# gmlwns2000/sea-attention

Measured on AMD Instinct MI355X. Metric: tokens/sec + achieved HBM GB/s, OPT-1.3B SEA T=4096 k=64, 1/2/4/8 MI355X, higher is better.
Workload: dtype bf16

## Files before the change

sea-attention_amd/csrc/sea_topk.hip:

```cpp
#include "sea_common.hpp"
#include "sea_tail.hpp"
#include "sea_convfrag.hpp"


#ifdef SEA_STAMP
__device__ unsigned long long sea_dbg[16];
#define STAMP(i) do { if (threadIdx.x == 0) { unsigned long long _t = __builtin_amdgcn_s_memtime(); \
  atomicAdd(&sea_dbg[i], _t - _tprev); _tprev = _t; } } while (0)
#else
#define STAMP(i) do {} while (0)
#endif

namespace sea {

constexpr int TK_THREADS = 256;
constexpr int TK_WAVES = TK_THREADS / WAVE;
constexpr int TK_MAX_BINS = 2048;

__device__ inline uint32_t f2key(float f) {
  f = f + 0.0f;
  uint32_t u = __float_as_uint(f);
  return u ^ ((u >> 31) ? 0xFFFFFFFFu : 0x80000000u);
}

struct TopkParams {
  const void* src;
  int64_t sn, sh, st;
  int H, T_dst, T_m, T_src;
  int is_causal, max_k;
  int M;
  int nchunks;
  int W;
  int G;
  const int32_t* keep;
  int64_t keep_stride_n;
  uint32_t* bits;
  float* mask_out;
  int32_t* row_nnz;
  int32_t* head_off;
  const int32_t* t_src_dev;
  int t_src_stride;
  int32_t* crow1;
};

template <typename T> __device__ inline void load4(const T* p, float* f);
template <> __device__ inline void load4<float>(const float* p, float* f) {
  float4 v = *reinterpret_cast<const float4*>(p);
  f[0] = v.x; f[1] = v.y; f[2] = v.z; f[3] = v.w;
}
template <> __device__ inline void load4<__hip_bfloat16>(const __hip_bfloat16* p, float* f) {
  uint2 v = *reinterpret_cast<const uint2*>(p);
  f[0] = __uint_as_float(v.x << 16); f[1] = __uint_as_float(v.x & 0xffff0000u);
  f[2] = __uint_as_float(v.y << 16); f[3] = __uint_as_float(v.y & 0xffff0000u);
}
template <> __device__ inline void load4<__half>(const __half* p, float* f) {
  uint2 v = *reinterpret_cast<const uint2*>(p);
  const __half2* h = reinterpret_cast<const __half2*>(&v);
  float2 a = __half22float2(h[0]), b = __half22float2(h[1]);
  f[0] = a.x; f[1] = a.y; f[2] = b.x; f[3] = b.y;
}

__device__ inline int block_excl_scan(int v, int* s_wave , int* total) {
  const int lane = threadIdx.x & 63, w = threadIdx.x >> 6;
  int incl = wave_incl_scan(v);
  if (lane == 63) s_wave[w] = incl;
  __syncthreads();
  int base = 0, tot = 0;
#pragma unroll
  for (int i = 0; i < TK_WAVES; ++i) {
    int x = s_wave[i];
    if (i < w) base += x;
    tot += x;
  }
  __syncthreads();
  *total = tot;
  return base + incl - v;
}

constexpr int TK_CAND_CAP = 1024;

template <typename T>
__device__ __noinline__ unsigned long long select_multipass(const T* base, int64_t sh, int T_m, int nchunks, int M, int K,
                                                            uint32_t umin, uint32_t umax, int rounds, int* s_hist,
                                                            int* s_wave, int* s_bcast) {
  const int tid = threadIdx.x;
  auto load_keys = [&](int j, uint32_t* k4) -> bool {
    const int c = j * TK_THREADS + tid;
    if (c >= nchunks) { k4[0] = k4[1] = k4[2] = k4[3] = 0u; return false; }
    const int f0 = c * 4;
    const int h = f0 / T_m, b0 = f0 - h * T_m;
    float f[4];
    load4<T>(base + h * sh + b0, f);
    for (int e = 0; e < 4; ++e) k4[e] = f2key(f[e]);
    return true;
  };
  unsigned long long sel = 0;
  uint32_t prefix = umax;
  int bits_left = (umax == umin) ? 0 : (32 - __clz(umax ^ umin));
  int kth = K, n_eq = M;
  while (bits_left > 0) {
    const int d = bits_left < 11 ? bits_left : 11;
    const int shift = bits_left - d;
    const int nb = 1 << d;
    const int hi = shift + d;
    for (int i = tid; i < nb; i += TK_THREADS) s_hist[i] = 0;
    __syncthreads();
    for (int j = 0; j < rounds; ++j) {
      uint32_t k4[4];
      if (!load_keys(j, k4)) continue;
      for (int e = 0; e < 4; ++e) {
        const uint32_t u = k4[e];
        const bool cand = (hi >= 32) ? true : ((u >> hi) == (prefix >> hi));
        if (cand) atomicAdd(&s_hist[nb - 1 - (int)((u >> shift) & (uint32_t)(nb - 1))], 1);
      }
    }
    __syncthreads();
    const int per = (nb + TK_THREADS - 1) / TK_THREADS;
    int mine = 0;
    for (int i = 0; i < per; ++i) {
      const int bi = tid * per + i;
      if (bi < nb) mine += s_hist[bi];
    }
    int total;
    const int excl = block_excl_scan(mine, s_wave, &total);
    if (excl < kth && kth <= excl + mine) {
      int run = excl;
      for (int i = 0; i < per; ++i) {
        const int bi = tid * per + i;
        const int c = s_hist[bi];
        if (kth <= run + c) { s_bcast[0] = bi; s_bcast[1] = run; s_bcast[2] = c; break; }
        run += c;
      }
    }
    __syncthreads();
    const int rb = s_bcast[0];
    kth -= s_bcast[1];
    n_eq = s_bcast[2];
    const uint32_t dmask = (uint32_t)(nb - 1) << shift;
    prefix = (prefix & ~dmask) | ((uint32_t)(nb - 1 - rb) << shift);
    bits_left = shift;
    __syncthreads();
  }
  const uint32_t tau = prefix;
  const int r = kth;
  int seen = 0;
  for (int j = 0; j < rounds; ++j) {
    uint32_t k4[4];
    const bool valid = load_keys(j, k4);
    int cnt = 0;
    for (int e = 0; e < 4; ++e) cnt += (valid && k4[e] == tau) ? 1 : 0;
    int total = 0, rank = 0;
    if (n_eq != r) rank = seen + block_excl_scan(cnt, s_wave, &total);
    for (int e = 0; e < 4; ++e) {
      if (!valid) continue;
      if (k4[e] > tau) sel |= 1ull << (4 * j + e);
      if (k4[e] == tau) {
        if (n_eq == r || rank < r) sel |= 1ull << (4 * j + e);
        ++rank;
      }
    }
    seen += total;
  }
  return sel;
}

__device__ inline long long block_excl_scan64(long long v, long long* s_wave , long long* total) {
  const int lane = threadIdx.x & 63, w = threadIdx.x >> 6;
  long long incl = wave_incl_scan(v);
  if (lane == 63) s_wave[w] = incl;
  __syncthreads();
  long long base = 0, tot = 0;
#pragma unroll
  for (int i = 0; i < TK_WAVES; ++i) {
    const long long x = s_wave[i];
    if (i < w) base += x;
    tot += x;
  }
  __syncthreads();
  *total = tot;
  return base + incl - v;
}

template <typename T, int EPT, bool FROM_MASK, bool FULL, int HMAX = 1024, bool EXT_CAND = false, bool K16 = false, bool HCW = K16>
__device__ __forceinline__ void select_body(const TopkParams& p, uint32_t (&key)[K16 ? EPT / 2 : EPT], unsigned long long sel, int n,
                                            int t, int row, const T* base, uint32_t* cand = nullptr) {
  constexpr int R = EPT / 4;
  static_assert(!K16 || (sizeof(T) == 2 && !FROM_MASK), "packed keys: 16-bit maps");
  auto key_at = [&](int i) -> uint32_t {
    if constexpr (K16) return (i & 1) ? (key[i >> 1] >> 16) : (key[i >> 1] & 0xffffu);
    else return key[i];
  };
  auto digit_at = [&](int i, int shift, int d) -> int {
    if constexpr (K16) return (int)__builtin_amdgcn_ubfe(~key[i >> 1], shift + 16 * (i & 1), d);
    else return (int)__builtin_amdgcn_ubfe(~key[i], shift, d);
  };
  __shared__ int s_hist[TK_MAX_BINS + 1];
  __shared__ int s_head[HMAX];
  __shared__ int s_wave[TK_WAVES];
  __shared__ uint32_t s_red[2 * TK_WAVES];
  __shared__ int s_bcast[4];
  uint32_t* s_ckey;
  uint32_t* s_cidx;
  if constexpr (EXT_CAND) {
    s_ckey = cand; s_cidx = cand + TK_CAND_CAP;
  } else {
    __shared__ uint32_t s_cand[2 * TK_CAND_CAP];
    s_ckey = s_cand; s_cidx = s_cand + TK_CAND_CAP;
  }
  __shared__ uint32_t s_selbits[512];
  __shared__ int s_ncand;

  const int tid = threadIdx.x;
  const int lane = tid & 63, wv = tid >> 6;
#ifdef SEA_STAMP
  unsigned long long _tprev = __builtin_amdgcn_s_memtime();
#endif
  for (int i = tid; i <= TK_MAX_BINS; i += TK_THREADS) s_hist[i] = 0;
  for (int i = tid; i < 512; i += TK_THREADS) s_selbits[i] = 0;
  for (int i = tid; i < p.H; i += TK_THREADS) s_head[i] = 0;
  if (tid == 0) s_ncand = 0;

  if (!FROM_MASK) {
    const int K = p.keep[n * p.keep_stride_n + t + (p.t_src_dev ? p.t_src_dev[n * p.t_src_stride] - p.T_dst : 0)];
    if (K >= p.M) {
#pragma unroll
      for (int j = 0; j < R; ++j)
        if (FULL || j * TK_THREADS + tid < p.nchunks) sel |= 0xFull << (4 * j);
      __syncthreads();
    } else if (K <= 0) {
      __syncthreads();
    } else {
      uint32_t umin = 0xFFFFFFFFu, umax = 0u;
      if constexpr (K16) {
        typedef unsigned short us2 __attribute__((ext_vector_type(2)));
        us2 mn = us2{0xFFFF, 0xFFFF}, mx = us2{0, 0};
#pragma unroll
        for (int j = 0; j < R; ++j) {
          if (FULL || j * TK_THREADS + tid < p.nchunks) {
            const us2 a = __builtin_bit_cast(us2, key[2 * j]), b = __builtin_bit_cast(us2, key[2 * j + 1]);
            mn = __builtin_elementwise_min(mn, __builtin_elementwise_min(a, b));
            mx = __builtin_elementwise_max(mx, __builtin_elementwise_max(a, b));
          }
        }
        umin = min((uint32_t)mn[0], (uint32_t)mn[1]);
        umax = max((uint32_t)mx[0], (uint32_t)mx[1]);
      } else {
#pragma unroll
      for (int j = 0; j < R; ++j) {
        if (FULL || j * TK_THREADS + tid < p.nchunks) {
          umin = min(umin, min(min(key[4 * j], key[4 * j + 1]), min(key[4 * j + 2], key[4 * j + 3])));
          umax = max(umax, max(max(key[4 * j], key[4 * j + 1]), max(key[4 * j + 2], key[4 * j + 3])));
        }
      }
      }
      umin = wave_min(umin);
      umax = wave_max(umax);
      if (lane == 0) { s_red[wv] = umin; s_red[TK_WAVES + wv] = umax; }
      __syncthreads();
#pragma unroll
      for (int i = 0; i < TK_WAVES; ++i) { umin = min(umin, s_red[i]); umax = max(umax, s_red[TK_WAVES + i]); }
      STAMP(1);
      const int bits_left = (umax == umin) ? 0 : (32 - __clz(umax ^ umin));
      bool fast = bits_left > 0;
      int rb_sel = 0, kth = K, c_in = 0, shift = 0, d = 0;
      if (fast) {
        d = bits_left < 11 ? bits_left : 11;
        shift = bits_left - d;
        const int nb = 1 << d;
#pragma unroll
        for (int i = 0; i < EPT; ++i) {
          int rb = digit_at(i, shift, d);
          if (!FULL) rb = (((i >> 2) * TK_THREADS + tid) < p.nchunks) ? rb : TK_MAX_BINS;
          atomicAdd(&s_hist[rb], 1);
        }
        __syncthreads();
        const int per = (nb + TK_THREADS - 1) / TK_THREADS;
        int mine = 0;
        for (int i = 0; i < per; ++i) {
          const int bi = tid * per + i;
          if (bi < nb) mine += s_hist[bi];
        }
        int total;
        const int excl = block_excl_scan(mine, s_wave, &total);
        if (excl < K && K <= excl + mine) {
          int run = excl;
          for (int i = 0; i < per; ++i) {
            const int bi = tid * per + i;
            const int c = s_hist[bi];
            if (K <= run + c) { s_bcast[0] = bi; s_bcast[1] = run; s_bcast[2] = c; break; }
            run += c;
          }
        }
        __syncthreads();
        rb_sel = s_bcast[0];
        kth = K - s_bcast[1];
        c_in = s_bcast[2];
        fast = c_in <= TK_CAND_CAP;
      }
      STAMP(2);
      if (fast) {
#pragma unroll
        for (int i = 0; i < EPT; ++i) {
          const int rb = digit_at(i, shift, d);
          const bool valid = FULL || (((i >> 2) * TK_THREADS + tid) < p.nchunks);
          if (valid && rb < rb_sel) sel |= 1ull << i;
          if (valid && rb == rb_sel) {
            const int slot = atomicAdd(&s_ncand, 1);
            s_ckey[slot] = key_at(i);
            s_cidx[slot] = (uint32_t)(((i >> 2) * TK_THREADS + tid) * 4 + (i & 3));
          }
        }
        __syncthreads();
        for (int ci = tid; ci < c_in; ci += TK_THREADS) {
          const uint32_t ku = s_ckey[ci], kf = s_cidx[ci];
          int rank = 0;
          for (int cj = 0; cj < c_in; ++cj) {
            const uint32_t ou = s_ckey[cj], of = s_cidx[cj];
            rank += (ou > ku || (ou == ku && of < kf)) ? 1 : 0;
          }
          if (rank < kth) atomicOr(&s_selbits[kf >> 5], 1u << (kf & 31));
        }
        __syncthreads();
#pragma unroll
        for (int j = 0; j < R; ++j) {
          const int c = j * TK_THREADS + tid;
          const unsigned long long nibx = (s_selbits[(c >> 3) & 511] >> (4 * (c & 7))) & 0xFu;
          sel |= nibx << (4 * j);
        }
      } else if constexpr (K16) {
        const bool hist = bits_left > 0;
        int n_eq = hist ? c_in : p.M;
        uint32_t tau_low = 0u;
        const uint32_t lowmask = hist ? ((1u << shift) - 1u) : 0u;
        auto in_bin = [&](int i) -> bool {
          const bool valid = FULL || (((i >> 2) * TK_THREADS + tid) < p.nchunks);
          return valid && (!hist || digit_at(i, shift, d) == rb_sel);
        };
        if (hist) {
#pragma unroll
          for (int i = 0; i < EPT; ++i) {
            const bool valid = FULL || (((i >> 2) * TK_THREADS + tid) < p.nchunks);
            if (valid && digit_at(i, shift, d) < rb_sel) sel |= 1ull << i;
          }
          if (shift > 0) {
            const int nb2 = 1 << shift;
            __syncthreads();
            if (tid < nb2) s_hist[tid] = 0;
            __syncthreads();
#pragma unroll
            for (int i = 0; i < EPT; ++i)
              if (in_bin(i)) atomicAdd(&s_hist[nb2 - 1 - (int)(key_at(i) & lowmask)], 1);
            __syncthreads();
            const int mine = tid < nb2 ? s_hist[tid] : 0;
            int total;
            const int excl = block_excl_scan(mine, s_wave, &total);
            if (tid < nb2 && excl < kth && kth <= excl + mine) { s_bcast[0] = tid; s_bcast[1] = excl; s_bcast[2] = mine; }
            __syncthreads();
            tau_low = (uint32_t)(nb2 - 1 - s_bcast[0]);
            kth -= s_bcast[1];
            n_eq = s_bcast[2];
#pragma unroll
            for (int i = 0; i < EPT; ++i)
              if (in_bin(i) && (key_at(i) & lowmask) > tau_low) sel |= 1ull << i;
          }
        }
        int seen = 0;
#pragma unroll
        for (int j = 0; j < R; ++j) {
          bool tie[4];
          int cnt = 0;
#pragma unroll
          for (int e = 0; e < 4; ++e) {
            tie[e] = in_bin(4 * j + e) && (key_at(4 * j + e) & lowmask) == tau_low;
            cnt += tie[e] ? 1 : 0;
          }
          int total = 0, rank = 0;
          if (n_eq != kth) rank = seen + block_excl_scan(cnt, s_wave, &total);
#pragma unroll
          for (int e = 0; e < 4; ++e) {
            if (tie[e]) {
              if (n_eq == kth || rank < kth) sel |= 1ull << (4 * j + e);
              ++rank;
            }
          }
          seen += total;
        }
        __syncthreads();
      } else {
        sel = select_multipass<T>(base, p.sh, p.T_m, p.nchunks, p.M, K, umin, umax, R, s_hist, s_wave, s_bcast);
        for (int i = tid; i < p.H; i += TK_THREADS) s_head[i] = 0;
        __syncthreads();
      }
    }
  } else {
    __syncthreads();
  }

  STAMP(3);
  const int w_t = row_width(t, p.T_dst, p.t_src_dev ? p.t_src_dev[n * p.t_src_stride] : p.T_src, p.is_causal);
  const float scale = interp_scale(w_t, p.T_m);
  const bool tm_pow2 = (p.T_m & (p.T_m - 1)) == 0;
  const int tm_sh = __ffs(p.T_m) - 1;
#pragma unroll
  for (int j = 0; j < R; ++j) {
    const int c = j * TK_THREADS + tid;
    const bool valid = FULL || c < p.nchunks;
    const uint32_t nib = (uint32_t)(sel >> (4 * j)) & 0xFu;
    uint32_t word = nib << (4 * (lane & 7));
    word |= dpp_u32<0xB1>(word);
    word |= dpp_u32<0x4E>(word);
    word |= dpp_u32<0x141>(word);
    if ((lane & 7) == 0 && (c >> 3) < p.W) p.bits[(int64_t)row * p.W + (c >> 3)] = word;
    if (p.mask_out != nullptr && valid) {
      const int f0 = c * 4;
      const int h = f0 / p.T_m, b0 = f0 - h * p.T_m;
      float4 m;
      m.x = (nib & 1u) ? 1.f : 0.f; m.y = (nib & 2u) ? 1.f : 0.f;
      m.z = (nib & 4u) ? 1.f : 0.f; m.w = (nib & 8u) ? 1.f : 0.f;
      *reinterpret_cast<float4*>(p.mask_out + (((int64_t)n * p.H + h) * p.T_dst + t) * p.T_m + b0) = m;
    }
  }
  if constexpr (K16 && HCW) {
    int wpx[4];
    {
      float bprev = interp_bound(4 * lane, scale);
#pragma unroll
      for (int e = 0; e < 4; ++e) {
        const float bnext = interp_bound(4 * lane + e + 1, scale);
        const int w = (int)(bnext - bprev);
        wpx[e] = w < p.max_k ? w : p.max_k;
        bprev = bnext;
      }
    }
#pragma unroll
    for (int j0 = 0; j0 < R; j0 += 8) {
      float red[8];
#pragma unroll
      for (int b = 0; b < 8; ++b) {
        int sum = 0;
        if (j0 + b < R) {
          const uint32_t nib = (uint32_t)(sel >> (4 * (j0 + b))) & 0xFu;
#pragma unroll
          for (int e = 0; e < 4; ++e) sum += (nib >> e) & 1u ? wpx[e] : 0;
        }
        red[b] = (float)sum;
      }
      const float x = wave_reduce8(red, [](float u, float v) { return u + v; });
#pragma unroll
      for (int b = 0; b < 8; ++b) {
        const int h = 4 * (j0 + b) + wv;
        if (j0 + b < R && h < p.H && lane == 0) s_head[h] = (int)reduce8_get(x, b);
      }
    }
  } else {
    unsigned long long m = sel;
    while (m) {
      const int i = __ffsll((long long)m) - 1;
      m &= m - 1;
      const int f = ((i >> 2) * TK_THREADS + tid) * 4 + (i & 3);
      const int h = tm_pow2 ? (f >> tm_sh) : f / p.T_m, b = f - h * p.T_m;
      int w = (int)(interp_bound(b + 1, scale) - interp_bound(b, scale));
      w = w < p.max_k ? w : p.max_k;
      if (w > 0) atomicAdd(&s_head[h], w);
    }
  }
  __syncthreads();
  STAMP(4);
  if (wv == 0) {
    int carry = 0;
    int32_t* ho = p.head_off + (int64_t)row * (p.H + 1);
    for (int h0 = 0; h0 < p.H; h0 += 64) {
      const int h = h0 + lane;
      const int v = h < p.H ? s_head[h] : 0;
      const int incl = wave_incl_scan(v);
      if (h < p.H) ho[h] = carry + incl - v;
      carry += __shfl(incl, 63);
    }
    if (lane == 0) {
      ho[p.H] = carry; p.row_nnz[row] = carry;
      if (p.crow1 != nullptr) { p.crow1[2 * row] = 0; p.crow1[2 * row + 1] = carry; }
    }
  }
}

template <typename T, int EPT, bool FROM_MASK, bool FULL>
__global__ __launch_bounds__(TK_THREADS) void topk_select_kernel(TopkParams p) {
  constexpr int R = EPT / 4;
  const int tid = threadIdx.x;
  const int row = blockIdx.x;
  const int n = row / p.T_dst, t = row - n * p.T_dst;
  const T* base = reinterpret_cast<const T*>(p.src) + n * p.sn + t * p.st;
#ifdef SEA_STAMP
  unsigned long long _tprev = __builtin_amdgcn_s_memtime();
#endif

  uint32_t key[EPT];
  unsigned long long sel = 0;
#pragma unroll
  for (int j = 0; j < R; ++j) {
    const int c = j * TK_THREADS + tid;
    float f[4] = {0.f, 0.f, 0.f, 0.f};
    const bool valid = FULL || c < p.nchunks;
    if (valid) {
      const int f0 = c * 4;
      const int h = f0 / p.T_m, b0 = f0 - h * p.T_m;
      load4<T>(base + h * p.sh + b0, f);
    }
#pragma unroll
    for (int e = 0; e < 4; ++e) {
      if (FROM_MASK) {
        if (valid && f[e] != 0.f) sel |= 1ull << (4 * j + e);
        key[4 * j + e] = 0;
      } else {
        key[4 * j + e] = valid ? f2key(f[e]) : 0u;
      }
    }
  }
  STAMP(0);
  select_body<T, EPT, FROM_MASK, FULL>(p, key, sel, n, t, row, base);
}

template <typename T, int EPT, bool FULL>
__device__ __forceinline__ void tail_select_row(const TailParams& tp, const TopkParams& p, float* s_z, int row) {
  constexpr int R = EPT / 4, E = 4;
  const int tid = threadIdx.x;
  const int lane = tid & 63;
  const int wv = __builtin_amdgcn_readfirstlane(tid >> 6);
  const int n = row / tp.T, t = row - n * tp.T;
  constexpr int LDZ = 64 + 3;
#ifdef SEA_STAMP
  unsigned long long _tprev = __builtin_amdgcn_s_memtime();
#endif
  uint32_t* s_tab = reinterpret_cast<uint32_t*>(s_z + ((tp.H + 15) / 16) * 16 * LDZ);
  TailRow<T, E> tr;
  if (tp.tab) tr.load_global(tp.tab, lane);
  tail_z_tile<T>(tp, s_z, n, t);
  if (!tp.tab) tail_consts_fill<T>(tp, s_tab, 64 * E);
  __syncthreads();
  if (!tp.tab) tr.load(s_tab, lane);
  STAMP(8);
  uint32_t key[EPT / 2];
  const int mine = FULL ? R : max(0, (tp.H - wv + 3) / 4);
  auto batch = [&](auto j0c, auto nbc) {
    constexpr int J0 = decltype(j0c)::value, NBC = decltype(nbc)::value;
    float a[NBC][E];
    const int nb = min(NBC, mine - J0);
    if (nb > 0) {
      tr.template heads_impl<true>(tp, lane, nb, [&](int b) { return s_z + (4 * (J0 + b) + wv) * LDZ; },
                                   [&](int b) { return (((int64_t)n * tp.H + (4 * (J0 + b) + wv)) * tp.T + t) * (64 * E); }, a);
    }
#pragma unroll
    for (int b = 0; b < NBC; ++b) {
      key[2 * (J0 + b)] = (b < nb) ? pack2<T>(a[b][0], a[b][1]) : 0u;
      key[2 * (J0 + b) + 1] = (b < nb) ? pack2<T>(a[b][2], a[b][3]) : 0u;
    }
  };
  static_assert(R <= 16, "two batches of eight heads per wave");
  if constexpr (R <= 8) {
    batch(std::integral_constant<int, 0>{}, std::integral_constant<int, R>{});
  } else {
    batch(std::integral_constant<int, 0>{}, std::integral_constant<int, 8>{});
    batch(std::integral_constant<int, 8>{}, std::integral_constant<int, R - 8>{});
  }
  STAMP(9);
  select_body<T, EPT, false, FULL, 64, true, true>(p, key, 0ull, n, t, row, (const T*)nullptr, reinterpret_cast<uint32_t*>(s_z));
}

template <typename T, int EPT, bool FULL>
#ifndef SEA_TSEL_OCC32
#define SEA_TSEL_OCC32 7
#endif
#ifndef SEA_TSEL_OCC16
#define SEA_TSEL_OCC16 7
#endif
__global__ __launch_bounds__(TK_THREADS, EPT <= 16 ? SEA_TSEL_OCC16 : EPT == 32 ? SEA_TSEL_OCC32 : EPT == 40 ? 5 : 1) void predictor_tail_select_kernel(TailParams tp, TopkParams p) {
  constexpr int R = EPT / 4, E = 4;
  extern __shared__ __attribute__((aligned(16))) float s_z[];
  const int tid = threadIdx.x;
  const int lane = tid & 63;
  const int wv = __builtin_amdgcn_readfirstlane(tid >> 6);
  const int row = blockIdx.x;
  const int n = row / tp.T, t = row - n * tp.T;
  constexpr int LDZ = 64 + 3;
#ifdef SEA_STAMP
  unsigned long long _tprev = __builtin_amdgcn_s_memtime();
#endif
  uint32_t* s_tab = reinterpret_cast<uint32_t*>(s_z + ((tp.H + 15) / 16) * 16 * LDZ);
  TailRow<T, E> tr;
  if (tp.tab) tr.load_global(tp.tab, lane);
  tail_z_tile<T>(tp, s_z, n, t);
  if (!tp.tab) tail_consts_fill<T>(tp, s_tab, 64 * E);
  __syncthreads();
  if (!tp.tab) tr.load(s_tab, lane);
  STAMP(8);
  uint32_t key[EPT / 2];
  const int mine = FULL ? R : max(0, (tp.H - wv + 3) / 4);
  auto batch = [&](auto j0c, auto nbc) {
    constexpr int J0 = decltype(j0c)::value, NBC = decltype(nbc)::value;
    float a[NBC][E];
    const int nb = min(NBC, mine - J0);
    if (nb > 0) {
      tr.template heads_impl<true>(tp, lane, nb, [&](int b) { return s_z + (4 * (J0 + b) + wv) * LDZ; },
                                   [&](int b) { return (((int64_t)n * tp.H + (4 * (J0 + b) + wv)) * tp.T + t) * (64 * E); }, a);
    }
#pragma unroll
    for (int b = 0; b < NBC; ++b) {
      key[2 * (J0 + b)] = (b < nb) ? pack2<T>(a[b][0], a[b][1]) : 0u;
      key[2 * (J0 + b) + 1] = (b < nb) ? pack2<T>(a[b][2], a[b][3]) : 0u;
    }
  };
  static_assert(R <= 16, "two batches of eight heads per wave");
  if constexpr (R <= 8) {
    batch(std::integral_constant<int, 0>{}, std::integral_constant<int, R>{});
  } else {
    batch(std::integral_constant<int, 0>{}, std::integral_constant<int, 8>{});
    batch(std::integral_constant<int, 8>{}, std::integral_constant<int, R - 8>{});
  }
  STAMP(9);
  select_body<T, EPT, false, FULL, 64, true, true>(p, key, 0ull, n, t, row, (const T*)nullptr, reinterpret_cast<uint32_t*>(s_z));
}

template <int EPT>
__global__ __launch_bounds__(TK_THREADS) void predictor_tail_select_f32_kernel(TailParams tp, TopkParams p) {
  using T = float;
  constexpr int R = EPT / 4, E = 4;
  extern __shared__ __attribute__((aligned(16))) float s_z[];
  const int tid = threadIdx.x;
  const int lane = tid & 63;
  const int wv = __builtin_amdgcn_readfirstlane(tid >> 6);
  const int row = blockIdx.x;
  const int n = row / tp.T, t = row - n * tp.T;
  constexpr int LDZ = 64 + 3;
  uint32_t* s_tab = reinterpret_cast<uint32_t*>(s_z + ((tp.H + 15) / 16) * 16 * LDZ);
  TailRow<T, E> tr;
  if (tp.tab) tr.load_global(tp.tab, lane);
  tail_z_tile<T>(tp, s_z, n, t);
  if (!tp.tab) tail_consts_fill<T>(tp, s_tab, 64 * E);
  __syncthreads();
  if (!tp.tab) tr.load(s_tab, lane);
  uint32_t key[EPT];
  const int mine = max(0, (tp.H - wv + 3) / 4);
  auto batch = [&](auto j0c, auto nbc) {
    constexpr int J0 = decltype(j0c)::value, NBC = decltype(nbc)::value;
    float a[NBC][E];
    const int nb = min(NBC, mine - J0);
    if (nb > 0) {
      tr.template heads_impl<true>(tp, lane, nb, [&](int b) { return s_z + (4 * (J0 + b) + wv) * LDZ; },
                                   [&](int b) { return (((int64_t)n * tp.H + (4 * (J0 + b) + wv)) * tp.T + t) * (64 * E); }, a);
    }
#pragma unroll
    for (int b = 0; b < NBC; ++b)
#pragma unroll
      for (int e = 0; e < E; ++e) key[4 * (J0 + b) + e] = (b < nb) ? f2key(a[b][e]) : 0u;
  };
  static_assert(R <= 8, "one batch of eight heads per wave (H <= 32)");
  batch(std::integral_constant<int, 0>{}, std::integral_constant<int, R>{});
  const T* base = reinterpret_cast<const T*>(tp.probs) + (int64_t)n * p.sn + (int64_t)t * p.st;
  select_body<T, EPT, false, false, 64, true, false, false>(p, key, 0ull, n, t, row, base, reinterpret_cast<uint32_t*>(s_z));
}

template <typename T, int E, int EPT>
__global__ __launch_bounds__(TK_THREADS) void predictor_tail_select_gen_kernel(TailParams tp, TopkParams p) {
  constexpr int R = EPT / 4;
  constexpr int NBC = E >= 6 ? 4 : 8;
  extern __shared__ __attribute__((aligned(16))) float s_z[];
  const int tid = threadIdx.x;
  const int lane = tid & 63;
  const int wv = __builtin_amdgcn_readfirstlane(tid >> 6);
  const int row = blockIdx.x;
  const int n = row / tp.T, t = row - n * tp.T;
  const int LDZ = tp.W4 + 3;
  uint32_t* s_tab = reinterpret_cast<uint32_t*>(s_z + ((tp.H + 15) / 16) * 16 * LDZ);
  const int zt_words = ((tp.H + 15) / 16) * 16 * LDZ + TAIL_TAB_ROWS * 64 * E;
  unsigned short* s_flat = reinterpret_cast<unsigned short*>(s_z + max(zt_words, 2 * TK_CAND_CAP));
  tail_z_tile<T>(tp, s_z, n, t);
  tail_consts_fill<T>(tp, s_tab, 64 * E);
  __syncthreads();
  TailRow<T, E> tr;
  tr.load(s_tab, lane);
  const int mine = max(0, (tp.H - wv + 3) / 4);
  for (int k0 = 0; k0 < mine; k0 += NBC) {
    float a[NBC][E];
    const int nb = min(NBC, mine - k0);
    tr.heads(tp, lane, nb, [&](int b) { return s_z + (wv + 4 * (k0 + b)) * LDZ; },
             [&](int b) { return (((int64_t)n * tp.H + (wv + 4 * (k0 + b))) * tp.T + t) * tp.T_M; }, a);
#pragma unroll
    for (int b = 0; b < NBC; ++b) {
      if (b < nb) {
        unsigned short* fr = s_flat + (wv + 4 * (k0 + b)) * tp.T_M + lane * E;
#pragma unroll
        for (int e = 0; e < E; ++e)
          if (lane * E + e < tp.T_M) fr[e] = __builtin_bit_cast(unsigned short, from_f<T>(a[b][e]));
      }
    }
  }
  __syncthreads();
  uint32_t key[EPT / 2];
#pragma unroll
  for (int j = 0; j < R; ++j) {
    const int c = j * TK_THREADS + tid;
    uint2 v = make_uint2(0u, 0u);
    if (c < p.nchunks) v = *reinterpret_cast<const uint2*>(s_flat + 4 * c);
    key[2 * j] = v.x;
    key[2 * j + 1] = v.y;
  }
  select_body<T, EPT, false, false, 64, true, true, false>(p, key, 0ull, n, t, row, (const T*)nullptr, reinterpret_cast<uint32_t*>(s_z));
}

template <typename I>
__global__ __launch_bounds__(1024) void row_scan_kernel(const int32_t* row_nnz, int T_dst, I* crow) {
  constexpr int PER = 16;
  __shared__ int s_w[2][16];
  const int n = blockIdx.x;
  const int tid = threadIdx.x, lane = tid & 63, w = tid >> 6;
  const int32_t* src = row_nnz + (int64_t)n * T_dst;
  I* dst = crow + (int64_t)n * (T_dst + 1);
  long long carry = 0;
  for (int t0 = 0; t0 < T_dst; t0 += 1024 * PER) {
    int vv[PER];
#pragma unroll
    for (int j = 0; j < PER; ++j) {
      const int t = t0 + j * 1024 + tid;
      vv[j] = t < T_dst ? src[t] : 0;
    }
#pragma unroll
    for (int j = 0; j < PER; ++j) {
      if (t0 + j * 1024 < T_dst) {
        const int t = t0 + j * 1024 + tid;
        const int v = vv[j];
        const int incl = wave_incl_scan(v);
        if (lane == 63) s_w[j & 1][w] = incl;
        __syncthreads();
        int base = 0, tot = 0;
#pragma unroll
        for (int i = 0; i < 16; ++i) { const int x = s_w[j & 1][i]; if (i < w) base += x; tot += x; }
        if (t < T_dst) dst[t] = (I)(carry + base + incl - v);
        carry += tot;
      }
    }
    __syncthreads();
  }
  if (tid == 0) dst[T_dst] = (I)carry;
}

struct EmitParams {
  const uint32_t* bits;
  const void* crow;
  int H, T_dst, T_m, T_src, is_causal, max_k, W;
// ... 814 lines not shown
```

Before: 15.74 million.

## Vectorize top-k candidate sweep with packed 16-bit compares and wave-aggregated slots

In the packed 16-bit key path, the per-element radix-digit candidate collection is replaced by SIMD packed-halfword subtraction sign tests. These build above and in-bin bitmasks, and a single wave-level atomic reserves candidate slots instead of one LDS atomic per element. It also zeroes shared histograms with 16-byte stores in one pass and computes per-head width sums with udot4 when max_k fits in a byte. The K16 path no longer writes mask_out, and the packed sweep is restricted to umax < 0x8000, falling back otherwise.

```diff
diff --git a/sea-attention_amd/csrc/sea_topk.hip b/sea-attention_amd/csrc/sea_topk.hip
--- a/sea-attention_amd/csrc/sea_topk.hip
+++ b/sea-attention_amd/csrc/sea_topk.hip
@@ -186,6 +186,7 @@
                                             int t, int row, const T* base, uint32_t* cand = nullptr) {
   constexpr int R = EPT / 4;
   static_assert(!K16 || (sizeof(T) == 2 && !FROM_MASK), "packed keys: 16-bit maps");
+  constexpr bool PKSWEEP = K16 && EPT >= 32;
   auto key_at = [&](int i) -> uint32_t {
     if constexpr (K16) return (i & 1) ? (key[i >> 1] >> 16) : (key[i >> 1] & 0xffffu);
     else return key[i];
@@ -194,8 +195,8 @@
     if constexpr (K16) return (int)__builtin_amdgcn_ubfe(~key[i >> 1], shift + 16 * (i & 1), d);
     else return (int)__builtin_amdgcn_ubfe(~key[i], shift, d);
   };
-  __shared__ int s_hist[TK_MAX_BINS + 1];
-  __shared__ int s_head[HMAX];
+  __shared__ __attribute__((aligned(16))) int s_hist[TK_MAX_BINS + 1];
+  __shared__ __attribute__((aligned(16))) int s_head[HMAX];
   __shared__ int s_wave[TK_WAVES];
   __shared__ uint32_t s_red[2 * TK_WAVES];
   __shared__ int s_bcast[4];
@@ -207,7 +208,7 @@
     __shared__ uint32_t s_cand[2 * TK_CAND_CAP];
     s_ckey = s_cand; s_cidx = s_cand + TK_CAND_CAP;
   }
-  __shared__ uint32_t s_selbits[512];
+  __shared__ __attribute__((aligned(16))) uint32_t s_selbits[512];
   __shared__ int s_ncand;
 
   const int tid = threadIdx.x;
@@ -215,10 +216,20 @@
 #ifdef SEA_STAMP
   unsigned long long _tprev = __builtin_amdgcn_s_memtime();
 #endif
+  if constexpr (K16 && HMAX == 64) {
+    static_assert(TK_MAX_BINS == 2 * 4 * TK_THREADS && TK_THREADS >= 128 + HMAX / 4 + 1, "one pass of 16-byte stores");
+    const uint4 z4 = make_uint4(0u, 0u, 0u, 0u);
+    reinterpret_cast<uint4*>(s_hist)[tid] = z4;
+    reinterpret_cast<uint4*>(s_hist)[TK_THREADS + tid] = z4;
+    if (tid < 128) reinterpret_cast<uint4*>(s_selbits)[tid] = z4;
+    else if (tid < 128 + HMAX / 4) reinterpret_cast<uint4*>(s_head)[tid - 128] = z4;
+    else if (tid == TK_THREADS - 1) { s_hist[TK_MAX_BINS] = 0; s_ncand = 0; }
+  } else {
   for (int i = tid; i <= TK_MAX_BINS; i += TK_THREADS) s_hist[i] = 0;
   for (int i = tid; i < 512; i += TK_THREADS) s_selbits[i] = 0;
   for (int i = tid; i < p.H; i += TK_THREADS) s_head[i] = 0;
   if (tid == 0) s_ncand = 0;
+  }
 
   if (!FROM_MASK) {
     const int K = p.keep[n * p.keep_stride_n + t + (p.t_src_dev ? p.t_src_dev[n * p.t_src_stride] - p.T_dst : 0)];
@@ -296,9 +307,68 @@
         kth = K - s_bcast[1];
         c_in = s_bcast[2];
         fast = c_in <= TK_CAND_CAP;
+        if constexpr (PKSWEEP) fast = fast && umax < 0x8000u;
       }
       STAMP(2);
       if (fast) {
+        if constexpr (PKSWEEP) {
+          typedef unsigned short us2 __attribute__((ext_vector_type(2)));
+          constexpr int NR = EPT / 2, NG = (NR + 15) / 16;
+          const uint32_t tB = ((umax >> bits_left) << bits_left) | ((uint32_t)((1 << d) - 1 - rb_sel) << shift);
+          const uint32_t tA = tB | ((1u << shift) - 1u);
+          const us2 ta2 = us2{(unsigned short)tA, (unsigned short)tA};
+          const us2 tb2 = us2{(unsigned short)(tB - 1u), (unsigned short)(tB - 1u)};
+          uint32_t inb[NG];
+          int nc = 0;
+#pragma unroll
+          for (int g = 0; g < NG; ++g) {
+            constexpr int G16 = 16;
+            const int nr = NR - G16 * g < G16 ? NR - G16 * g : G16;
+            uint32_t ab = 0u, le = 0u, vm = 0u;
+#pragma unroll
+            for (int r = 0; r < G16; ++r) {
+              if (r < nr) {
+                const us2 kk = __builtin_bit_cast(us2, key[G16 * g + r]);
+                ab = (ab >> 1) | (__builtin_bit_cast(uint32_t, ta2 - kk) & 0x80008000u);
+                le = (le >> 1) | (__builtin_bit_cast(uint32_t, tb2 - kk) & 0x80008000u);
+                if (!FULL && (r & 1) == 0 && (((G16 * g + r) >> 1) * TK_THREADS + tid) < p.nchunks) vm |= 0x00030003u << r;
+              }
+            }
+            ab >>= G16 - nr; le >>= G16 - nr;
+            if (!FULL) { ab &= vm; le &= vm; }
+            inb[g] = le & ~ab;
+            nc += __popc(inb[g]);
+            auto spread = [](uint32_t x) -> uint32_t {
+              x = (x | (x << 8)) & 0x00FF00FFu;
+              x = (x | (x << 4)) & 0x0F0F0F0Fu;
+              x = (x | (x << 2)) & 0x33333333u;
+              return (x | (x << 1)) & 0x55555555u;
+            };
+            sel |= (unsigned long long)(spread(ab & 0xFFFFu) | (spread(ab >> 16) << 1)) << (32 * g);
+          }
+          if (__builtin_amdgcn_ballot_w64(nc != 0) != 0ull) {
+            const int incl = wave_incl_scan(nc);
+            const int wtot = __builtin_amdgcn_readlane(incl, 63);
+            int wbase = 0;
+            if (lane == 0) wbase = atomicAdd(&s_ncand, wtot);
+            int slot = __builtin_amdgcn_readfirstlane(wbase) + incl - nc;
+#pragma unroll
+            for (int g = 0; g < NG; ++g) {
+#pragma unroll
+              for (int r = 0; r < 16; ++r) {
+                if (16 * g + r < NR) {
+                  const uint32_t m = inb[g] & (0x00010001u << r);
+                  if (__builtin_amdgcn_ballot_w64(m != 0u) != 0ull) {
+                    const int i0 = 2 * (16 * g + r);
+                    const uint32_t f0 = (uint32_t)(((i0 >> 2) * TK_THREADS + tid) * 4 + (i0 & 3));
+                    if (m & 0xFFFFu) { s_ckey[slot] = key[16 * g + r] & 0xFFFFu; s_cidx[slot] = f0; ++slot; }
+                    if (m >> 16) { s_ckey[slot] = key[16 * g + r] >> 16; s_cidx[slot] = f0 + 1u; ++slot; }
+                  }
+                }
+              }
+            }
+          }
+        } else {
 #pragma unroll
         for (int i = 0; i < EPT; ++i) {
           const int rb = digit_at(i, shift, d);
@@ -309,6 +379,7 @@
             s_ckey[slot] = key_at(i);
             s_cidx[slot] = (uint32_t)(((i >> 2) * TK_THREADS + tid) * 4 + (i & 3));
           }
+        }
         }
         __syncthreads();
         for (int ci = tid; ci < c_in; ci += TK_THREADS) {
@@ -411,6 +482,7 @@
     word |= dpp_u32<0x4E>(word);
     word |= dpp_u32<0x141>(word);
     if ((lane & 7) == 0 && (c >> 3) < p.W) p.bits[(int64_t)row * p.W + (c >> 3)] = word;
+    if constexpr (!K16)
     if (p.mask_out != nullptr && valid) {
       const int f0 = c * 4;
       const int h = f0 / p.T_m, b0 = f0 - h * p.T_m;
@@ -432,18 +504,27 @@
         bprev = bnext;
       }
     }
+    const bool w8 = p.max_k <= 255;
+    const uint32_t wpk = (uint32_t)wpx[0] | ((uint32_t)wpx[1] << 8) | ((uint32_t)wpx[2] << 16) | ((uint32_t)wpx[3] << 24);
 #pragma unroll
     for (int j0 = 0; j0 < R; j0 += 8) {
       float red[8];
-#pragma unroll
-      for (int b = 0; b < 8; ++b) {
-        int sum = 0;
-        if (j0 + b < R) {
-          const uint32_t nib = (uint32_t)(sel >> (4 * (j0 + b))) & 0xFu;
-#pragma unroll
-          for (int e = 0; e < 4; ++e) sum += (nib >> e) & 1u ? wpx[e] : 0;
+      auto nib_at = [&](int b) -> uint32_t { return (uint32_t)(sel >> (4 * (j0 + b))) & 0xFu; };
+      if (w8) {
+#pragma unroll
+        for (int b = 0; b < 8; ++b)
+          red[b] = j0 + b < R ? (float)__builtin_amdgcn_udot4((nib_at(b) * 0x00204081u) & 0x01010101u, wpk, 0u, false) : 0.f;
+      } else {
+#pragma unroll
+        for (int b = 0; b < 8; ++b) {
+          int sum = 0;
+          if (j0 + b < R) {
+            const uint32_t nib = nib_at(b);
+#pragma unroll
+            for (int e = 0; e < 4; ++e) sum += (nib >> e) & 1u ? wpx[e] : 0;
+          }
+          red[b] = (float)sum;
         }
-        red[b] = (float)sum;
       }
       const float x = wave_reduce8(red, [](float u, float v) { return u + v; });
 #pragma unroll
```

Result: no change. 15.80 million, median of 6 (+0.4%).
